# huang-yh/SelfOcc

Hardware: AMD Instinct MI355X
Metric: rendered rays/sec (6-cam 450x800, 128 samples/ray) (higher is better)
Workload: dtype f32; 1 GPU; BASELINE configs[1]: 6 cams x 450x800 rays, 128 samples/ray, volume 200x200x16; volume_channels=1, feat_storage=f32, preheat_steps=150

## Files before the change

selfocc_amd/csrc/render_fwd.hip:

```cpp
#include "so_device.h"
#include "sh_device.h"
#include "ray_device.h"

template <int NF, bool BF16>
int so_render_fwd_samples(const so_render_args &a, hipStream_t st);
template <int NB>
int so_render_sh_samples(const so_render_args &a, hipStream_t st);

namespace {

SO_DEVFN RayGeom so_pixel_ray(const so_render_args &a, int cam, int ix, int iy) {
    typedef const __attribute__((address_space(4))) float *so_const_fptr;
    const so_const_fptr M = (so_const_fptr)(a.img2lidar + cam * 16);
    float u = (float)ix * a.sx + a.ox;
    float v = (float)iy * a.sy + a.oy;
    RayGeom g;
    g.ox = M[3]; g.oy = M[7]; g.oz = M[11];
    float dx = (M[0] * u + M[1] * v) + M[2];
    float dy = (M[4] * u + M[5] * v) + M[6];
    float dz = (M[8] * u + M[9] * v) + M[10];
    g.dn = sqrtf((dx * dx + dy * dy) + dz * dz);
    g.dx = dx / g.dn; g.dy = dy / g.dn; g.dz = dz / g.dn;
    return g;
}
// ... 568 lines not shown
            gvd = fmaf(fh, e1 - e0, e0);
            gvh = dh0;

            const float cosv = fmaf(gvd, Gdd, fmaf(gvw, Gdw, gvh * Gdh));
            const float alpha = so_alpha_fast(sdf * s2, fminf(cosv, 0.0f) * hdt_s2);
            w = alpha * T;
            T = T * ((1.0f - alpha) + 1e-7f);
        }

        const float t_mid = fmaf(fi, dt, tnear + hdt);
        acc = acc + w;
        dsum = fmaf(w, t_mid, dsum);
        if (w > best_w) { best_w = w; best_t = t_mid; }

        if constexpr (NF > 0) {
            so_cell c;
            c.h0 = st.h0; c.w0 = st.w0; c.d0 = st.d0;
            float wk[8];
            const float fh = st.fh, fw = st.fw, fd = st.fd;
            const float fh0 = 1.0f - fh, fw0 = 1.0f - fw, fd0 = 1.0f - fd;
            const float ww0 = fw0 * fh0, ww1 = fw * fh0, ww2 = fw0 * fh, ww3 = fw * fh;
            wk[0] = fd0 * ww0; wk[1] = fd * ww0; wk[2] = fd0 * ww1; wk[3] = fd * ww1;
            wk[4] = fd0 * ww2; wk[5] = fd * ww2; wk[6] = fd0 * ww3; wk[7] = fd * ww3;
            float f[NF];
            bool done = false;
            if constexpr (STAGED) {
                if (st.boxed) {
                    so_gather_feat_staged<NF, BF16>(rf, a.feat_vol, H, W, D, st.h0, st.w0, st.d0, st.hmin, st.wmin,
                                                    st.dmin, wk, lds, lane, lane_vox, st.pref, st.blk,
                                                    st.all_interior, f);
                    done = true;
                }
            }
            if (!done) {
                if (st.all_interior) so_gather_feat_interior<NF, BF16>(rf, W, D, st.cell, wk, f);
                else so_gather_feat<NF, BF16>(a.feat_vol, H, W, D, c, wk, f);
            }
#pragma unroll
            for (int k = 0; k < 3; ++k) {
                float col = fmaxf(fmaf(0.28209479177387814f, f[k], 0.5f), 0.0f);
                rgb[k] = fmaf(w, col, rgb[k]);
            }
            if constexpr (NSEM > 0) {
                float m = f[3];
#pragma unroll
                for (int k = 1; k < NSEM; ++k) m = fmaxf(m, f[3 + k]);
                float e[NSEM], den = 0.0f;
#pragma unroll
                for (int k = 0; k < NSEM; ++k) {
                    e[k] = so_fast_exp2((f[3 + k] - m) * 1.44269504088896341f);
                    den = den + e[k];
                }
                const float wd = w * so_fast_rcp(den);
                if constexpr (SEM_LDS) {
#pragma unroll
                    for (int k = 0; k < NSEM; ++k) sem_lds[k * 256] = fmaf(wd, e[k], sem_lds[k * 256]);
                } else {
#pragma unroll
                    for (int k = 0; k < NSEM; ++k) sem[k] = fmaf(wd, e[k], sem[k]);
                }
            }
        }
    };

    if constexpr (PIPE) {
        FastStep<NF> A, B;
        fetch(0, A);
        for (int i = 0;;) {
            if (i + 1 < S) fetch(i + 1, B);
            consume(i, A);
            if (++i >= S) break;
            if (so_all(T < 1e-10f)) break;
            if (i + 1 < S) fetch(i + 1, A);
            consume(i, B);
            if (++i >= S) break;
            if (so_all(T < 1e-10f)) break;
        }
    } else {
        for (int i = 0; i < S; ++i) {
            FastStep<NF> A;
            fetch(i, A);
            consume(i, A);
            if (so_all(T < 1e-10f)) break;
        }
    }

    const float eps32 = 1.1920928955078125e-07f;
    if (dt * inv_dn < eps32) best_t = tnear + hdt;
    if (!store) return;
    float depth = dsum * so_fast_rcp(acc + 1e-10f);
    if (a.flags & SO_FLAG_DEPTH_DIV_NORM) depth = depth * inv_dn;
    if (a.depth) a.depth[ray] = depth;
    if (a.acc) a.acc[ray] = acc;
    if (a.max_depth) a.max_depth[ray] = best_t * inv_dn;
    if (a.nears) a.nears[ray] = tnear;
    if (a.fars) a.fars[ray] = tfar;
    if constexpr (NF > 0) {
        if (a.rgb) {
#pragma unroll
            for (int k = 0; k < 3; ++k) {
                float bg = 0.0f;
                if (a.bkgd_mode == SO_BKGD_CONST) bg = a.bkgd[k];
                else if (a.bkgd_mode == SO_BKGD_PER_RAY) bg = a.bkgd_rays[3 * (size_t)ray + k];
                float r = rgb[k];
                if (a.bkgd_mode != SO_BKGD_NONE) r = r + bg * (1.0f - acc);
                if (a.flags & SO_FLAG_CLAMP_RGB) r = fminf(fmaxf(r, 0.0f), 1.0f);
                a.rgb[3 * (size_t)ray + k] = r;
            }
        }
        if constexpr (NSEM > 0) {
            if (a.sem) {
#pragma unroll
                for (int k = 0; k < NSEM; ++k) a.sem[(size_t)ray * NSEM + k] = SEM_LDS ? sem_lds[k * 256] : sem[k];
            }
        }
    }
}

constexpr int kRunExitFreeSteps = 60000;
constexpr int kSureScan = 8;

struct AheadStep {
    float gh, gw, gd, fi;
    int h0, w0, d0;
    unsigned cell, code;
    bool all_interior;
};

template <bool FACE_SAFE, class GeomFn>
SO_DEVFN void so_march_fast_ahead(const so_render_args &a, int ray, GeomFn geom) {
    const int H = a.map.h.tot_len, W = a.map.w.tot_len, D = a.map.d.tot_len;
    const int S = a.n_samples;
    const RayGeom g = geom(a);
    float tnear, tfar;
    so_collide(a, g, tnear, tfar);
    const float dt = (tfar - tnear) / (float)S;
    const float inv_dn = 1.0f / g.dn;
    const AxisK kh = so_axis_affine(a.map.h), kw = so_axis_affine(a.map.w), kd = so_axis_affine(a.map.d);
    const float t_off = (a.sample_pos == SO_SAMPLE_AT_START) ? tnear : tnear + 0.5f * dt;
    const float Gdh = g.dy * kh.k1, Gdw = g.dx * kw.k1, Gdd = g.dz * kd.k1;
    const float G0h = fmaf(g.oy, kh.k1, kh.k0) + Gdh * t_off;
    const float G0w = fmaf(g.ox, kw.k1, kw.k0) + Gdw * t_off;
    const float G0d = fmaf(g.oz, kd.k1, kd.k0) + Gdd * t_off;
    const float s2 = so_inv_s(a) * 1.44269504088896341f;
    const float hdt = 0.5f * dt, hdt_s2 = hdt * s2;
    const float *__restrict__ vol = a.sdf_vol;
    const unsigned n_cells = (unsigned)(H * W * D);
    const __amdgpu_buffer_rsrc_t rb = so_make_rsrc(a.sdf_brick, (size_t)n_cells * 17);
    const __amdgpu_buffer_rsrc_t rs = so_make_rsrc(vol, (size_t)n_cells * 4);
    const int rcode = max((int)ceilf(dt / so_skip_unit(a.aabb, S)), 1);
    const int maxdim = max(H, max(W, D));
    const float face_m = 3.0f * 1.1920929e-7f * (float)(1u << (32 - __builtin_clz((unsigned)maxdim)));

    float T = 1.0f, acc = 0.0f, dsum = 0.0f, best_w = -1.0f, best_t = 0.0f;

    auto place = [&](const int i, AheadStep &st) __attribute__((always_inline)) {
        st.fi = (float)i;
        const float step = st.fi * dt;
        const float gh = fmaf(Gdh, step, G0h), gw = fmaf(Gdw, step, G0w), gd = fmaf(Gdd, step, G0d);
        st.gh = gh; st.gw = gw; st.gd = gd;
        const int h0 = so_floor_i(gh), w0 = so_floor_i(gw), d0 = so_floor_i(gd);
        st.h0 = h0; st.w0 = w0; st.d0 = d0;
        st.cell = so_cell_index(h0, w0, d0, W, D);
    };
    auto interior = [&](const AheadStep &st) __attribute__((always_inline)) {
        return so_all3((unsigned)st.h0 < (unsigned)(H - 1), (unsigned)st.w0 < (unsigned)(W - 1), (unsigned)st.d0 < (unsigned)(D - 1));
    };
    int i_lo = S, i_hi = -1;
    {
        AheadStep p;
        const int n = min(kSureScan, S);
#pragma nounroll
        for (int k = 0; k < n; ++k) {
            place(k, p);
            if (interior(p)) { i_lo = k; break; }
        }
        if (i_lo < S) {
#pragma nounroll
            for (int k = S - 1; k >= S - n && k >= i_lo; --k) {
                place(k, p);
                if (interior(p)) { i_hi = k; break; }
            }
        }
        if (i_hi < 0) i_lo = S;
    }
    auto sure = [&](const int i) __attribute__((always_inline)) { return i >= i_lo && i <= i_hi; };

    auto locate = [&](const int i, AheadStep &st) __attribute__((always_inline)) {
        place(i, st);
        st.all_interior = true;
        if (!sure(i)) st.all_interior = interior(st);
        st.code = 0u;
        if (st.all_interior) st.code = __builtin_amdgcn_raw_buffer_load_b8(rb, st.cell, n_cells * 16u, 0);
    };
    auto near_face = [&](float fh, float fw, float fd) __attribute__((always_inline)) {
        return fmaxf(fmaxf(fabsf(fh - 0.5f), fabsf(fw - 0.5f)), fabsf(fd - 0.5f)) > 0.5f - face_m;
    };
    auto canon_cell = [&](const int i) __attribute__((always_inline)) {
        const RayGeom gc = geom(so_reload_args());
        __builtin_amdgcn_sched_barrier(0);
        float px, py, pz;
        {
            const so_render_args ac = so_reload_args();
            const int n = ac.n_samples;
            const float b0 = so_bin(i, n);
            const float t_start = b0 * tfar + (1.0f - b0) * tnear;
            if (ac.sample_pos == SO_SAMPLE_AT_START) {
                px = gc.ox + gc.dx * t_start; py = gc.oy + gc.dy * t_start; pz = gc.oz + gc.dz * t_start;
            } else {
                const float b1 = so_bin(i + 1, n);
                const float tt = t_start + (b1 * tfar + (1.0f - b1) * tnear);
                px = gc.ox + (gc.dx * tt) / 2.0f; py = gc.oy + (gc.dy * tt) / 2.0f; pz = gc.oz + (gc.dz * tt) / 2.0f;
            }
        }
        __builtin_amdgcn_sched_barrier(0);
        float slope;
        const float gh = so_grid_coord(so_axis_m2g(so_reload_args().map.h, py, slope), so_reload_args().map.h.tot_len);
        __builtin_amdgcn_sched_barrier(0);
        const float gw = so_grid_coord(so_axis_m2g(so_reload_args().map.w, px, slope), so_reload_args().map.w.tot_len);
        __builtin_amdgcn_sched_barrier(0);
        const float gd = so_grid_coord(so_axis_m2g(so_reload_args().map.d, pz, slope), so_reload_args().map.d.tot_len);
        return so_cell_of(gh, gw, gd);
    };

    auto step = [&](const int i, AheadStep &cur, AheadStep &nxt) __attribute__((always_inline)) {
        const bool skip = cur.all_interior && so_all((int)cur.code >= rcode);
        if (i + 1 < S) locate(i + 1, nxt);
        float w;
        if (skip) {
            w = kAlphaFree * T;
            T = T * ((1.0f - kAlphaFree) + 1e-7f);
        } else {
            float fh = __builtin_amdgcn_fractf(cur.gh), fw = __builtin_amdgcn_fractf(cur.gw), fd = __builtin_amdgcn_fractf(cur.gd);
            so_f32x2 p0, p1, p2, p3;
            auto gather = [&](int h0, int w0, int d0) __attribute__((always_inline)) {
                float v[8];
                so_gather_sdf_buf(rs, H, W, D, h0, w0, d0, v);
                p0 = so_f32x2{v[0], v[4]}; p1 = so_f32x2{v[1], v[5]}; p2 = so_f32x2{v[2], v[6]}; p3 = so_f32x2{v[3], v[7]};
            };
            bool loaded = false;
            if constexpr (FACE_SAFE) {
                if (__any(near_face(fh, fw, fd))) {
                    int h0 = cur.h0, w0 = cur.w0, d0 = cur.d0;
                    bool moved = false;
                    if (near_face(fh, fw, fd)) {
                        const so_cell c = canon_cell(i);
                        if (c.h0 != h0 || c.w0 != w0 || c.d0 != d0) {
                            h0 = c.h0; w0 = c.w0; d0 = c.d0;
                            fh = c.fh1; fw = c.fw1; fd = c.fd1;
                            moved = true;
                        }
                    }
                    if (__any(moved)) { gather(h0, w0, d0); loaded = true; }
                }
            }
            if (!loaded) {
                if (cur.all_interior) {
                    {
                        const so_f4v lo = so_bload4(rb, cur.cell * 16u, 0u), hi = so_bload4(rb, cur.cell * 16u, (unsigned)D * 16u);
                        p0 = lo.xy; p1 = lo.zw; p2 = hi.xy; p3 = hi.zw;
                    }
                } else {
                    gather(cur.h0, cur.w0, cur.d0);
                }
            }
            float sdf, dh0, gvw, gvd;
            so_trilerp_fast_pk(p0, p1, p2, p3, fh, fw, fd, sdf, dh0, gvw, gvd);
            const float cosv = fmaf(gvd, Gdd, fmaf(gvw, Gdw, dh0 * Gdh));
            const float alpha = so_alpha_fast(sdf * s2, fminf(cosv, 0.0f) * hdt_s2);
            w = alpha * T;
            T = T * ((1.0f - alpha) + 1e-7f);
        }
        const float t_mid = fmaf(cur.fi, dt, tnear + hdt);
        acc = acc + w;
        dsum = fmaf(w, t_mid, dsum);
        if (w > best_w) { best_w = w; best_t = t_mid; }
        return skip;
    };

    auto run = [&](int &i, AheadStep &st) __attribute__((always_inline)) {
        if (i < i_lo || i >= i_hi) return false;
        auto free_step = [&]() __attribute__((always_inline)) {
            const float t_mid = fmaf(st.fi, dt, tnear + hdt);
            ++i;
            place(i, st);
            st.all_interior = true;
            st.code = __builtin_amdgcn_raw_buffer_load_b8(rb, st.cell, n_cells * 16u, 0);
            const float w = kAlphaFree * T;
            T = T * ((1.0f - kAlphaFree) + 1e-7f);
            acc = acc + w;
            dsum = fmaf(w, t_mid, dsum);
        };
        if (S <= kRunExitFreeSteps && !so_all(T < 2e-10f)) {
            while (i < i_hi && so_all((int)st.code >= rcode)) free_step();
        } else {
            while (i < i_hi && so_all((int)st.code >= rcode)) {
                free_step();
                if (so_all(T < 1e-10f)) return true;
            }
        }
        return false;
    };

    {
        AheadStep A, B;
        locate(0, A);
        for (int i = 0;;) {
            const bool sa = step(i, A, B);
            if (++i >= S) break;
            if (so_all(T < 1e-10f)) break;
            if (sa && run(i, B)) break;
            const bool sb = step(i, B, A);
            if (++i >= S) break;
            if (so_all(T < 1e-10f)) break;
            if (sb && run(i, A)) break;
        }
    }

    const float eps32 = 1.1920928955078125e-07f;
    if (dt * inv_dn < eps32) best_t = tnear + hdt;
    float depth = dsum * so_fast_rcp(acc + 1e-10f);
    if (a.flags & SO_FLAG_DEPTH_DIV_NORM) depth = depth * inv_dn;
    if (a.depth) a.depth[ray] = depth;
    if (a.acc) a.acc[ray] = acc;
    if (a.max_depth) a.max_depth[ray] = best_t * inv_dn;
    if (a.nears) a.nears[ray] = tnear;
    if (a.fars) a.fars[ray] = tfar;
}

enum class March {
    Canonical,
    Fast,
    FastFaceSafe,
    Skip,
    SkipFaceSafe,
    CanonicalUpscale,
};
constexpr bool so_is_fast(March m) { return m == March::Fast || m == March::FastFaceSafe; }
constexpr bool so_is_skip(March m) { return m == March::Skip || m == March::SkipFaceSafe; }
constexpr bool so_face_safe(March m) { return m == March::FastFaceSafe || m == March::SkipFaceSafe; }
template <int NF, bool BF16>
constexpr bool so_is_staged(March m) { return so_is_fast(m) && !BF16 && NF >= 4; }

template <int NF, bool BF16, March MODE, class GeomFn>
SO_DEVFN void so_march(const so_render_args &a, int ray, GeomFn geom) {
    if constexpr (MODE == March::CanonicalUpscale) {
        so_march_exact<NF, BF16, SO_MAP_UPSCALE>(a, ray, geom(a));
    } else if constexpr (so_is_skip(MODE)) {
        static_assert(NF == 0, "skip marcher: SDF-only launches");
        so_march_fast_ahead<so_face_safe(MODE)>(a, ray, geom);
    } else if constexpr (so_is_fast(MODE)) {
        so_march_fast<NF, BF16, false, so_face_safe(MODE)>(a, ray, geom);
    } else {
        so_march_exact<NF, BF16>(a, ray, geom(a));
    }
}


__global__ __launch_bounds__(256) void sdf_brickify_kernel(const float *__restrict__ vol, float *__restrict__ brick,
                                                           int H, int W, int D, so_render_args a, int with_codes) {
    const int h = blockIdx.x, h1 = min(h + 1, H - 1);
    const size_t n_cells = (size_t)H * W * D;
    uint8_t *codes = (uint8_t *)(brick + n_cells * 4);
    const bool quads = (D & 3) == 0 && (blockDim.x & 3) == 0;
    const float kd = a.map.d.size0 / a.map.d.range0, kw = a.map.w.size0 / a.map.w.range0, kh = a.map.h.size0 / a.map.h.range0;
    for (int w = blockIdx.y * blockDim.y + threadIdx.y; w < W; w += gridDim.y * blockDim.y) {
        const int w1 = min(w + 1, W - 1);
        const float *r00 = vol + ((size_t)h * W + w) * D, *r01 = vol + ((size_t)h * W + w1) * D;
        const float *r10 = vol + ((size_t)h1 * W + w) * D, *r11 = vol + ((size_t)h1 * W + w1) * D;
        for (int d = threadIdx.x; d < D; d += blockDim.x) {
            const int d1 = min(d + 1, D - 1);
            const float v0 = r00[d], v1 = r00[d1], v2 = r01[d], v3 = r01[d1];
            const float v4 = r10[d], v5 = r10[d1], v6 = r11[d], v7 = r11[d1];
            const size_t cell = ((size_t)h * W + w) * D + d;
            ((float4 *)brick)[cell] = make_float4(v0, v4, v1, v5);
            unsigned code = 0u;
            if (with_codes) {
                const float m = fminf(fminf(fminf(v0, v1), fminf(v2, v3)), fminf(fminf(v4, v5), fminf(v6, v7)));
                const float gd = fmaxf(fmaxf(fabsf(v1 - v0), fabsf(v3 - v2)), fmaxf(fabsf(v5 - v4), fabsf(v7 - v6))) * kd;
                const float gw = fmaxf(fmaxf(fabsf(v2 - v0), fabsf(v3 - v1)), fmaxf(fabsf(v6 - v4), fabsf(v7 - v5))) * kw;
                const float gh = fmaxf(fmaxf(fabsf(v4 - v0), fabsf(v5 - v1)), fmaxf(fabsf(v6 - v2), fabsf(v7 - v3))) * kh;
                const float G = sqrtf((gd * gd + gw * gw) + gh * gh) * 1.001f + 1e-20f;
                const float slack = m - kSkipArg / so_inv_s(a);
                if (slack > 0.0f && so_inv_s(a) > 0.0f) {
                    const float allow = 2.0f * slack / G / so_skip_unit(a.aabb, a.n_samples);
                    code = (unsigned)fminf(floorf(allow * 0.999f), 255.0f);
                }
            }
            if (quads) {
                const unsigned c1 = (unsigned)__builtin_amdgcn_update_dpp(0, (int)code, 0x55, 0xf, 0xf, false);
                const unsigned c2 = (unsigned)__builtin_amdgcn_update_dpp(0, (int)code, 0xaa, 0xf, 0xf, false);
                const unsigned c3 = (unsigned)__builtin_amdgcn_update_dpp(0, (int)code, 0xff, 0xf, 0xf, false);
                if ((d & 3) == 0) *(unsigned *)(codes + cell) = code | (c1 << 8) | (c2 << 16) | (c3 << 24);
            } else {
                codes[cell] = (uint8_t)code;
            }
        }
    }
}

struct TilePixel { int cam, ix, iy, wave, lane; };
SO_DEVFN TilePixel so_tile_pixel(int tiles_x, int tiles_y) {
    const int b = blockIdx.x;
    const int cam = b / (tiles_x * tiles_y);
    const int tb = b - cam * tiles_x * tiles_y;
    const int ty = tb / tiles_x, tx = tb - ty * tiles_x;
    const int wave = threadIdx.x >> 6, lane = threadIdx.x & 63;
    return {cam, tx * 16 + (wave & 1) * 8 + (lane & 7), ty * 16 + (wave >> 1) * 8 + (lane >> 3), wave, lane};
}

template <int NF, bool BF16, March MODE>
__global__ __launch_bounds__(256, (NF >= 8 ? 2 : 1)) void render_fwd_explicit(so_render_args a) {
    int ray = blockIdx.x * blockDim.x + threadIdx.x;
    if (ray >= a.n_rays) return;
    auto geom = [&](const so_render_args &a) __attribute__((always_inline)) { return so_explicit_ray(a, ray); };
    so_march<NF, BF16, MODE>(a, ray, geom);
}

template <int NF, bool BF16, March MODE>
SO_DEVFN void pixgrid_body(const so_render_args &a, int tiles_x, int tiles_y) {
    const TilePixel p = so_tile_pixel(tiles_x, tiles_y);
    const int cam = p.cam, wave = p.wave, lane = p.lane;
    int ix = p.ix, iy = p.iy;
    if constexpr (so_is_staged<NF, BF16>(MODE)) {
        __shared__ __attribute__((aligned(16))) float s_stage[4 * StageGeom<NF>::kWaveDwords];
        const bool real = (ix < a.nx) && (iy < a.ny);
        ix = min(ix, a.nx - 1); iy = min(iy, a.ny - 1);
        int ray = (cam * a.ny + iy) * a.nx + ix;
        auto geom = [&](const so_render_args &a) __attribute__((always_inline)) { return so_pixel_ray(a, cam, ix, iy); };
        constexpr int NSEM_LDS = NF - 3 >= 16 ? NF - 3 : 0;
        __shared__ float s_sem[NSEM_LDS > 0 ? NSEM_LDS * 256 : 1];
        so_march_fast<NF, BF16, true, so_face_safe(MODE)>(a, ray, geom, real, s_stage + wave * StageGeom<NF>::kWaveDwords, lane,
                                                          s_sem + threadIdx.x);
    } else {
        if (ix >= a.nx || iy >= a.ny) return;
        int ray = (cam * a.ny + iy) * a.nx + ix;
        auto geom = [&](const so_render_args &a) __attribute__((always_inline)) { return so_pixel_ray(a, cam, ix, iy); };
        so_march<NF, BF16, MODE>(a, ray, geom);
    }
}

template <int NF, bool BF16, March MODE>
__global__ __launch_bounds__(256, (NF >= 8 ? 2 : 1)) void render_fwd_pixgrid(so_render_args a, int tiles_x, int tiles_y) {
    pixgrid_body<NF, BF16, MODE>(a, tiles_x, tiles_y);
}
template <>
__global__ __launch_bounds__(256, 1) __attribute__((amdgpu_num_sgpr(80))) void render_fwd_pixgrid<0, false, March::Skip>(
    so_render_args a, int tiles_x, int tiles_y) {
    pixgrid_body<0, false, March::Skip>(a, tiles_x, tiles_y);
}
template <>
__global__ __launch_bounds__(256, 1) __attribute__((amdgpu_num_sgpr(80))) void render_fwd_pixgrid<0, false, March::SkipFaceSafe>(
    so_render_args a, int tiles_x, int tiles_y) {
    pixgrid_body<0, false, March::SkipFaceSafe>(a, tiles_x, tiles_y);
}

template <int NF, bool BF16, March MODE>
int launch_fwd(const so_render_args &a, hipStream_t st) {
    if (a.ray_mode == SO_RAYS_EXPLICIT) {
        int blocks = (a.n_rays + 255) / 256;
        hipLaunchKernelGGL((render_fwd_explicit<NF, BF16, MODE>), dim3(blocks), dim3(256), 0, st, a);
    } else {
        int tiles_x = (a.nx + 15) / 16, tiles_y = (a.ny + 15) / 16;
        int blocks = tiles_x * tiles_y * a.n_cams;
        hipLaunchKernelGGL((render_fwd_pixgrid<NF, BF16, MODE>), dim3(blocks), dim3(256), 0, st, a, tiles_x, tiles_y);
    }
    return so_launch_status();
}

template <int NF, bool BF16>
int dispatch_ps(const so_render_args &a, hipStream_t st) {
    bool per_sample = a.weights || a.ts || a.deltas || a.sdf || a.grad;
    if (per_sample) return so_render_fwd_samples<NF, BF16>(a, st);
    if (a.map.kind == SO_MAP_UPSCALE) {
        if constexpr (NF == 24 && BF16) {
            SO_REQUIRE(false, "the 'linear_upscale' mapping is built for n_rgb + n_sem = 0, 3, 8 and float32 24 (got bfloat16 24)");
        } else {
            return launch_fwd<NF, BF16, March::CanonicalUpscale>(a, st);
        }
    }
    bool fast = !(a.flags & SO_FLAG_EXACT) && a.jitter_mode == SO_JITTER_NONE && a.map.kind == SO_MAP_LINEAR &&
                a.map.h.size1 == 0.0f && a.map.w.size1 == 0.0f && a.map.d.size1 == 0.0f &&
                (long long)a.map.h.tot_len * a.map.w.tot_len < (1 << 24) && a.map.d.tot_len < (1 << 24);
    if (fast) {
        if (a.sdf_brick) {
            const int with_codes = (NF == 0 && !(a.flags & SO_FLAG_NO_SKIP)) ? 1 : 0;
            const int H = a.map.h.tot_len, W = a.map.w.tot_len, D = a.map.d.tot_len;
            int qx = 1;
            while (qx < D && qx < 256) qx *= 2;
            const int wy = 256 / qx;
            hipLaunchKernelGGL(sdf_brickify_kernel, dim3(H, min((W + wy - 1) / wy, 65535)), dim3(qx, wy), 0, st, a.sdf_vol, a.sdf_brick,
                               H, W, D, a, with_codes);
        }
        if constexpr (NF == 0) {
            if (a.sdf_brick && !(a.flags & (SO_FLAG_NO_SKIP | SO_FLAG_NO_AHEAD)))
                return (a.flags & SO_FLAG_NO_FACE_SAFE) ? launch_fwd<0, false, March::Skip>(a, st) : launch_fwd<0, false, March::SkipFaceSafe>(a, st);
        }
        if (!(a.flags & SO_FLAG_NO_FACE_SAFE)) return launch_fwd<NF, BF16, March::FastFaceSafe>(a, st);
        return launch_fwd<NF, BF16, March::Fast>(a, st);
    }
    return launch_fwd<NF, BF16, March::Canonical>(a, st);
}

template <int NB, int MK>
__global__ __launch_bounds__(256) void render_sh_explicit(so_render_args a) {
    const int ray = blockIdx.x * blockDim.x + threadIdx.x;
    if (ray >= a.n_rays) return;
    so_march_exact<so_sh_stride(NB), false, MK, NB>(a, ray, so_explicit_ray(a, ray));
}

template <int NB, int MK>
__global__ __launch_bounds__(256) void render_sh_pixgrid(so_render_args a, int tiles_x, int tiles_y) {
    const int b = blockIdx.x;
    const int cam = b / (tiles_x * tiles_y);
    const int tb = b - cam * tiles_x * tiles_y;
    const int ty = tb / tiles_x, tx = tb - ty * tiles_x;
    const int wave = threadIdx.x >> 6, lane = threadIdx.x & 63;
    const int ix = tx * 16 + (wave & 1) * 8 + (lane & 7);
    const int iy = ty * 16 + (wave >> 1) * 8 + (lane >> 3);
    if (ix >= a.nx || iy >= a.ny) return;
    const int ray = (cam * a.ny + iy) * a.nx + ix;
    so_march_exact<so_sh_stride(NB), false, MK, NB>(a, ray, so_pixel_ray(a, cam, ix, iy));
}

template <int NB, int MK>
int launch_sh(const so_render_args &a, hipStream_t st) {
    if (a.ray_mode == SO_RAYS_EXPLICIT) {
        hipLaunchKernelGGL((render_sh_explicit<NB, MK>), dim3((a.n_rays + 255) / 256), dim3(256), 0, st, a);
    } else {
        const int tiles_x = (a.nx + 15) / 16, tiles_y = (a.ny + 15) / 16;
        hipLaunchKernelGGL((render_sh_pixgrid<NB, MK>), dim3(tiles_x * tiles_y * a.n_cams), dim3(256), 0, st, a, tiles_x, tiles_y);
    }
    return so_launch_status();
}

template <int NB>
int dispatch_sh(const so_render_args &a, hipStream_t st) {
    if (a.weights || a.ts || a.deltas || a.sdf || a.grad) return so_render_sh_samples<NB>(a, st);
    return a.map.kind == SO_MAP_UPSCALE ? launch_sh<NB, SO_MAP_UPSCALE>(a, st) : launch_sh<NB, SO_MAP_LINEAR>(a, st);
}

}

int so_validate_mapping(const so_mapping &m) {
    SO_REQUIRE(m.kind == SO_MAP_LINEAR || m.kind == SO_MAP_UPSCALE, "mapping: unknown kind %d (0 = linear, 1 = linear_upscale)",
               (int)m.kind);
    const so_axis *ax[3] = {&m.h, &m.w, &m.d};
    const so_upscale_axis *ux[3] = {&m.uh, &m.uw, &m.ud};
    for (int i = 0; i < 3; ++i) {
        SO_REQUIRE(ax[i]->tot_len >= 2, "mapping axis %d: tot_len must be >= 2", i);
        SO_REQUIRE(ax[i]->size0 > 0 && ax[i]->range0 > 0, "mapping axis %d: size0/range0 must be > 0", i);
        if (m.kind == SO_MAP_LINEAR) {
            SO_REQUIRE(ax[i]->size1 == 0 || ax[i]->range1 > 0, "mapping axis %d: range1 must be > 0", i);
        } else {
            SO_REQUIRE(ax[i]->size1 >= 1, "linear_upscale axis %d: outer cells must be >= 1 (got %g)", i, (double)ax[i]->size1);
            SO_REQUIRE(ux[i]->unit > 0 && __builtin_isfinite(ux[i]->unit), "linear_upscale axis %d: unit must be > 0 (got %g)", i,
                       (double)ux[i]->unit);
            SO_REQUIRE(ux[i]->inc > 0 && __builtin_isfinite(ux[i]->inc),
                       "linear_upscale axis %d: increase unit must be > 0 (got %g): the outer range must exceed outer * unit",
                       i, (double)ux[i]->inc);
        }
    }
    return 0;
}

namespace {
template <int MK>
__global__ __launch_bounds__(256) void meter2grid_kernel(so_mapping m, const float *__restrict__ xyz, int n, int normalize,
                                                         float *__restrict__ hwd) {
    const int i = blockIdx.x * blockDim.x + threadIdx.x;
    if (i >= n) return;
    float gh, gw, gd, sh, sw, sd;
    so_m2g<MK>(m, xyz[3 * (size_t)i], xyz[3 * (size_t)i + 1], xyz[3 * (size_t)i + 2], gh, gw, gd, sh, sw, sd);
    if (normalize) {
        gh = gh / (float)(m.h.tot_len - 1); gw = gw / (float)(m.w.tot_len - 1); gd = gd / (float)(m.d.tot_len - 1);
    }
    hwd[3 * (size_t)i] = gh; hwd[3 * (size_t)i + 1] = gw; hwd[3 * (size_t)i + 2] = gd;
}
}

extern "C" int selfocc_meter2grid(const so_mapping *map, const float *xyz, int n, int normalize, float *hwd, void *stream) {
    SO_REQUIRE(map != nullptr, "map is NULL");
    if (so_validate_mapping(*map)) return -1;
    SO_REQUIRE(n >= 0, "n must be >= 0");
    if (n == 0) return 0;
    SO_REQUIRE(xyz != nullptr && hwd != nullptr, "xyz / hwd is NULL");
    const dim3 grid((unsigned)((n + 255) / 256));
    if (map->kind == SO_MAP_UPSCALE)
        hipLaunchKernelGGL(meter2grid_kernel<SO_MAP_UPSCALE>, grid, dim3(256), 0, (hipStream_t)stream, *map, xyz, n, normalize, hwd);
    else
        hipLaunchKernelGGL(meter2grid_kernel<SO_MAP_LINEAR>, grid, dim3(256), 0, (hipStream_t)stream, *map, xyz, n, normalize, hwd);
    return so_launch_status();
}

int so_validate_render(const so_render_args &a) {
    if (so_validate_mapping(a.map)) return -1;
    SO_REQUIRE(a.sdf_vol != nullptr, "sdf_vol is NULL");
    SO_REQUIRE(a.n_samples >= 1, "n_samples must be >= 1");
    SO_REQUIRE(a.n_rays >= 0, "n_rays must be >= 0");
    SO_REQUIRE(a.n_rgb == 0 || a.n_rgb == 3, "n_rgb must be 0 or 3 (the colour outputs; sh_deg sets the coefficient count)");
    SO_REQUIRE(a.n_sem >= 0, "n_sem must be >= 0");
    SO_REQUIRE(a.n_sem == 0 || a.n_rgb == 3, "semantic channels require n_rgb == 3");
    SO_REQUIRE(a.sh_deg >= 0 && a.sh_deg <= 2, "sh_deg %d is not built (built: sh_deg 0, 1, 2)", (int)a.sh_deg);
    SO_REQUIRE(a.sh_act == SO_SH_RELU || a.sh_act == SO_SH_SIGMOID, "sh_act %d is unknown (0 = relu, 1 = sigmoid)", (int)a.sh_act);
    if (a.n_rgb + a.n_sem > 0) {
        SO_REQUIRE(a.feat_vol != nullptr, "feat_vol is NULL but n_rgb + n_sem > 0");
        SO_REQUIRE(a.feat_dtype == SO_DTYPE_F32 || a.feat_dtype == SO_DTYPE_BF16, "bad feat_dtype");
        SO_REQUIRE(a.feat_stride % 4 == 0 && a.feat_stride >= a.n_rgb + a.n_sem,
                   "feat_stride must be a multiple of 4 and >= n_rgb + n_sem");
    }
    if (so_sh_launch(a)) {
        const int n_coef = 3 * (a.sh_deg + 1) * (a.sh_deg + 1);
        SO_REQUIRE(a.n_sem == 0, "sh_deg > 0 / sh_act = sigmoid with n_sem = %d semantic channels is not built (built: n_sem = 0)",
                   (int)a.n_sem);
        SO_REQUIRE(a.feat_dtype == SO_DTYPE_F32, "sh_deg > 0 / sh_act = sigmoid with a bfloat16 feature volume is not built (built: float32)");
        SO_REQUIRE(a.feat_stride == ((n_coef + 3) & ~3), "sh_deg = %d reads %d coefficients: feat_stride must be %d (got %d)",
                   (int)a.sh_deg, n_coef, (n_coef + 3) & ~3, (int)a.feat_stride);
    }
// ... 41 lines not shown
```

Measured before the change: 6.818 billion rays/s.

## Add tight full-sample inner loop for non-free cells in ray march

Adds a full_run loop that keeps marching through occupied cells in a tight inline loop: it issues the next cell's code load, then does the trilinear SDF/gradient fetch and alpha compositing. The main loop is restructured from an unrolled A/B ping-pong into cur/nxt with a struct copy, and branches to either the free-space run or the new full run. This is meant to cut per-step loop overhead and branching. In exchange it adds register pressure and code size, and the AheadStep copy on every step.

```diff
diff --git a/selfocc_amd/csrc/render_fwd.hip b/selfocc_amd/csrc/render_fwd.hip
--- a/selfocc_amd/csrc/render_fwd.hip
+++ b/selfocc_amd/csrc/render_fwd.hip
@@ -894,18 +894,45 @@
         return false;
     };
 
+    auto full_run = [&](int &i, AheadStep &st) __attribute__((always_inline)) {
+        if (i < i_lo) return false;
+        while (i < i_hi) {
+            if (so_all((int)st.code >= rcode)) return false;
+            const float fh = __builtin_amdgcn_fractf(st.gh), fw = __builtin_amdgcn_fractf(st.gw), fd = __builtin_amdgcn_fractf(st.gd);
+            if constexpr (FACE_SAFE) {
+                if (__any(near_face(fh, fw, fd))) return false;
+            }
+            const unsigned rec = st.cell * 16u;
+            const float t_mid = fmaf(st.fi, dt, tnear + hdt);
+            ++i;
+            place(i, st);
+            st.all_interior = true;
+            st.code = __builtin_amdgcn_raw_buffer_load_b8(rb, st.cell, n_cells * 16u, 0);
+            __builtin_amdgcn_sched_barrier(0);
+            const so_f4v lo = so_bload4(rb, rec, 0u), hi = so_bload4(rb, rec, (unsigned)D * 16u);
+            float sdf, dh0, gvw, gvd;
+            so_trilerp_fast_pk(lo.xy, lo.zw, hi.xy, hi.zw, fh, fw, fd, sdf, dh0, gvw, gvd);
+            const float cosv = fmaf(gvd, Gdd, fmaf(gvw, Gdw, dh0 * Gdh));
+            const float alpha = so_alpha_fast(sdf * s2, fminf(cosv, 0.0f) * hdt_s2);
+            const float w = alpha * T;
+            T = T * ((1.0f - alpha) + 1e-7f);
+            acc = acc + w;
+            dsum = fmaf(w, t_mid, dsum);
+            if (w > best_w) { best_w = w; best_t = t_mid; }
+            if (so_all(T < 1e-10f)) return true;
+        }
+        return false;
+    };
+
     {
-        AheadStep A, B;
-        locate(0, A);
+        AheadStep cur, nxt;
+        locate(0, cur);
         for (int i = 0;;) {
-            const bool sa = step(i, A, B);
+            const bool skipped = step(i, cur, nxt);
             if (++i >= S) break;
             if (so_all(T < 1e-10f)) break;
-            if (sa && run(i, B)) break;
-            const bool sb = step(i, B, A);
-            if (++i >= S) break;
-            if (so_all(T < 1e-10f)) break;
-            if (sb && run(i, A)) break;
+            if (skipped ? run(i, nxt) : full_run(i, nxt)) break;
+            cur = nxt;
         }
     }
 
```

After: 6.967 billion rays/s (median of 6 runs). +2.2%, better.
